# theoad/ot-vae-lightning

Measured on AMD Instinct MI355X. Metric: training images/sec (whole node) + OT-loss rel-err vs CPU ref, higher is better.
Workload: dtype f32; 1 GPU; MNIST-32 CNN VAE (capacity 8, latent 128x1x1, residual=add) + GaussianPrior(loss_coeff=0.1): fwd+bwd+Adam + latent Gaussian statistics update, hipGraph replay; per_gpu_batch=1024, global_batch=1024, parallelism=single GPU

## Files before the change

ot_vae_lightning_amd/csrc/attention.hip:

```cpp
#include "common.h"
#include <type_traits>

#define LOG2E 1.4426950408889634f
#define LN2 0.6931471805599453f
#define EXP2(x) __builtin_amdgcn_exp2f(x)
#define ATTN_LDS_FLOATS 16384
#ifndef OTVAE_ATTN_PACK
#define OTVAE_ATTN_PACK 1
#endif
#define ATTN_BOUND_GAP 64.0f

template <int C>
__device__ __forceinline__ float dotc(const float (&a)[C], const float* __restrict__ b) {
    float s = 0.f;
#pragma unroll
    for (int c = 0; c < C; ++c) s = fmaf(a[c], b[c], s);
    return s;
}

template <int C>
struct Rec {
    static constexpr int KV = 2 * C;
    static constexpr int QG = (2 * C + 2 + 3) & ~3;
};

__device__ __forceinline__ int adiv(int k, int d, float inv_d) {
    return k < (1 << 22) ? (int)(((float)k + 0.5f) * inv_d) : k / d;
}

template <int C, int STRIDE = 2 * C>
__device__ __forceinline__ void stage_kv(float* __restrict__ sm, const float* __restrict__ qkv, long slice0, int nsl, int T,
                                         int H) {
    const int HC = H * C, W3 = 3 * HC;
    const int per = T * 2 * C;
    const float inv_per = 1.0f / (float)per, inv_h = 1.0f / (float)H;
    const int n0 = (int)(slice0 / H), h0 = (int)(slice0 - (long)n0 * H);
    const int total = nsl * per, NT = blockDim.x;
    for (int e0 = threadIdx.x; e0 < total; e0 += 4 * NT) {
        float val[4];
        int dst[4];
#pragma unroll
        for (int u = 0; u < 4; ++u) {
            const int e = e0 + u * NT;
            dst[u] = -1;
            val[u] = 0.f;
            if (e < total) {
                const int sl = adiv(e, per, inv_per), r = e - sl * per;
                const int t = r / (2 * C), j = r - t * 2 * C;
                const int which = j / C, c = j - which * C;
                const int hs = h0 + sl;
                const int dn = adiv(hs, H, inv_h);
                const long n = n0 + dn;
                const int h = hs - dn * H;
                dst[u] = STRIDE == 2 * C ? e : (sl * T + t) * STRIDE + j;
// ... 134 lines not shown
                    const float wv = w[ci * ncols + j];
#pragma unroll
                    for (int t = 0; t < 4; ++t) a[t][j] = fmaf(xr[t], wv, a[t][j]);
                }
            }
        }
        store(tg * 4, col, a);
    }
}

template <int C, int KVS, int NC, bool QREC, bool AFF = false>
__device__ __forceinline__ void stage_qkv(float* __restrict__ kvrec, float* __restrict__ qd, int qstride, float qmul,
                                          const float* __restrict__ xs, const float* __restrict__ wl, int ntok, int T, int H,
                                          float* __restrict__ gq, const float* __restrict__ sc = nullptr,
                                          const float* __restrict__ sh = nullptr) {
    const int HC = H * C, W3 = 3 * HC;
    token_gemm<NC, AFF>(xs, ntok, HC, wl, W3, [&](int t0_, int col0, const float (&a)[4][NC]) {
        const int img = t0_ / T, tt = t0_ - img * T;
#pragma unroll
        for (int j = 0; j < NC; ++j) {
            const int col = col0 + j;
            const int part = col / HC, hc = col - part * HC;
            const int h_ = hc / C, c_ = hc - h_ * C;
            float* dst;
            int stride;
            float mul = 1.f;
            if (part == 0) {
                if constexpr (QREC) {
                    dst = qd + ((size_t)(img * H + h_) * T + tt) * qstride + c_;
                    stride = qstride;
                } else {
                    dst = qd + (size_t)t0_ * HC + hc;
                    stride = HC;
                }
                mul = qmul;
            } else {
                dst = kvrec + ((size_t)(img * H + h_) * T + tt) * KVS + (part - 1) * C + c_;
                stride = KVS;
            }
#pragma unroll
            for (int t = 0; t < 4; ++t) dst[t * stride] = a[t][j] * mul;
        }
        if (gq) {
#pragma unroll
            for (int t = 0; t < 4; ++t) {
                float* g = gq + (size_t)(t0_ + t) * W3 + col0;
                if constexpr (NC == 2) *reinterpret_cast<float2*>(g) = make_float2(a[t][0], a[t][1]);
                else g[0] = a[t][0];
            }
        }
    }, sc, sh);
}

template <int NC>
__device__ __forceinline__ void column_sums_to_partial(double (&s1)[NC], double (&s2)[NC], double* __restrict__ red, int HC,
                                                       double* __restrict__ partial) {
    const int cg = HC / NC;
    for (int m = cg; m < 64; m <<= 1) {
#pragma unroll
        for (int j = 0; j < NC; ++j) {
            s1[j] += __shfl_xor(s1[j], m, 64);
            s2[j] += __shfl_xor(s2[j], m, 64);
        }
    }
    const int lane = threadIdx.x & 63, wave = threadIdx.x >> 6, nw = blockDim.x >> 6;
    if (lane < cg) {
#pragma unroll
        for (int j = 0; j < NC; ++j) {
            red[(wave * 2 + 0) * HC + lane * NC + j] = s1[j];
            red[(wave * 2 + 1) * HC + lane * NC + j] = s2[j];
        }
    }
    __syncthreads();
    if ((int)threadIdx.x < 2 * HC) {
        const int which = threadIdx.x / HC, cc = threadIdx.x - which * HC;
        double t = red[which * HC + cc];
        for (int w = 1; w < nw; ++w) t += red[(w * 2 + which) * HC + cc];
        bn_stat_out(partial, which, HC, cc, gridDim.x, blockIdx.x, t);
    }
}

template <int NC>
__device__ __forceinline__ void stage_project(const float* __restrict__ xs, const float* __restrict__ wl, double* __restrict__ red,
                                              int ntok, int HC, float* __restrict__ yg, const float* __restrict__ rg,
                                              double* __restrict__ stat_partial) {
    double s1[NC], s2[NC];
#pragma unroll
    for (int j = 0; j < NC; ++j) s1[j] = s2[j] = 0.;
    token_gemm<NC>(xs, ntok, HC, wl, HC, [&](int t0_, int col0, const float (&a)[4][NC]) {
#pragma unroll
        for (int t = 0; t < 4; ++t) {
            const size_t o = (size_t)(t0_ + t) * HC + col0;
            float v[NC];
#pragma unroll
            for (int j = 0; j < NC; ++j) v[j] = a[t][j];
            if (rg) {
                if constexpr (NC == 2) {
                    const float2 rv = *reinterpret_cast<const float2*>(rg + o);
                    v[0] += rv.x, v[1] += rv.y;
                } else v[0] += rg[o];
            }
            if constexpr (NC == 2) *reinterpret_cast<float2*>(yg + o) = make_float2(v[0], v[1]);
            else yg[o] = v[0];
#pragma unroll
            for (int j = 0; j < NC; ++j) {
                s1[j] += (double)v[j];
                s2[j] += (double)v[j] * (double)v[j];
            }
        }
    });
    if (stat_partial) column_sums_to_partial<NC>(s1, s2, red, HC, stat_partial);
}

template <int C, int QPT, bool AUX, bool FUSED>
__device__ __forceinline__ void attn_fwd_body(float* __restrict__ sm, const float* __restrict__ qkv, int N, int T, int H, int SPB,
                                              float* __restrict__ out, float* __restrict__ lse, float* __restrict__ aux,
                                              float qk_scale, const AttnStage& sg) {
    constexpr int KVS = FwdRec<C, AUX>::KV;
    const int HC = H * C, W3 = 3 * HC;
    const int TPS = T / QPT;
    const long total = (long)N * H;
    const long slice0 = (long)blockIdx.x * SPB;
    const int nsl = (int)min((long)SPB, total - slice0);
    float* qs = sm + (size_t)SPB * T * KVS;
    float* xs = qs + (size_t)SPB * T * C;
    float* wl = xs + (size_t)SPB * T * C;
    float* wpl = wl + 3 * HC * HC;
    const int ntok = FUSED ? nsl / H * T : 0;
    const size_t tok0 = FUSED ? (size_t)(slice0 / H) * T : 0;
    if constexpr (FUSED) {
        if (sg.fold.slots) {
            __shared__ __align__(16) float bn_tab[2][32];
            bn_fold_prologue(sg.fold, HC, bn_tab[0], bn_tab[1], blockIdx.x == 0);
            stage_input_tile(xs, sg.x + tok0 * HC, ntok * HC, HC, bn_tab[0], bn_tab[1]);
        } else {
            stage_input_tile(xs, sg.x + tok0 * HC, ntok * HC, HC, sg.scale, sg.shift);
        }
        stage_weights(wl, sg.wqkv, HC * W3);
        stage_weights(wpl, sg.wproj, HC * HC);
        __syncthreads();
        float* gq = sg.qkv ? sg.qkv + tok0 * W3 : nullptr;
        if (HC & 1) stage_qkv<C, KVS, 1, false>(sm, qs, 0, 1.f, xs, wl, ntok, T, H, gq);
        else stage_qkv<C, KVS, 2, false>(sm, qs, 0, 1.f, xs, wl, ntok, T, H, gq);
    } else {
        stage_kv<C, KVS>(sm, qkv, slice0, nsl, T, H);
    }
    __syncthreads();
    const int sl = adiv((int)threadIdx.x, TPS, 1.0f / (float)TPS);
    const bool active = sl < nsl;
    const int t0 = (threadIdx.x - sl * TPS) * QPT;
    long n;
    int h;
    {
        const int bn0 = (int)(slice0 / H), bh0 = (int)(slice0 - (long)bn0 * H);
        const int hs = bh0 + sl;
        const int dn = adiv(hs, H, 1.0f / (float)H);
        n = bn0 + dn;
        h = hs - dn * H;
    }
    const float inv_c = LOG2E * qk_scale;
    float* kv = sm + (size_t)(active ? sl : 0) * T * KVS;

    constexpr int NA = AUX ? C * C + C : 1;
    float q[QPT][C], acc[QPT][C], mx[QPT], l[QPT], am[QPT][NA];
    __shared__ float red[4];
    const bool fast = slice_reduce_ok(TPS);
    float vbar[C], kmax = -INFINITY, kmin = INFINITY, knorm = 0.f;
#pragma unroll
    for (int c = 0; c < C; ++c) vbar[c] = 0.f;
    if (fast) {
#pragma unroll
        for (int i = 0; i < QPT; ++i) {
            const float* r = kv + (size_t)(t0 + i) * KVS;
            if constexpr (AUX) {
#pragma unroll
                for (int c = 0; c < C; ++c) vbar[c] += r[C + c];
            }
            if constexpr (C == 1) {
                kmax = fmaxf(kmax, r[0]);
                kmin = fminf(kmin, r[0]);
            } else {
                float s2 = 0.f;
#pragma unroll
                for (int c = 0; c < C; ++c) s2 = fmaf(r[c], r[c], s2);
                knorm = fmaxf(knorm, s2);
            }
        }
        if constexpr (C > 1) knorm = __builtin_sqrtf(slice_reduce<1>(knorm, TPS, red));
        if constexpr (AUX) {
#pragma unroll
            for (int c = 0; c < C; ++c) vbar[c] = slice_reduce<0>(vbar[c], TPS, red);
        }
// ... 121 lines not shown
                f2 sc = nm2[j];
#pragma unroll
                for (int c = 0; c < C; ++c) sc = __builtin_elementwise_fma(q2[j][c], (f2){kk[c], kk[c]}, sc);
                scs[2 * j] = sc.x;
                scs[2 * j + 1] = sc.y;
            }
        } else {
#pragma unroll
            for (int i = 0; i < QPT; ++i) {
                float sc = -mx[i];
#pragma unroll
                for (int c = 0; c < C; ++c) sc = fmaf(q[i][c], kk[c], sc);
                scs[i] = sc;
            }
        }
#pragma unroll
        for (int i = 0; i < QPT; ++i) {
            const float p = EXP2(scs[i]);
            l[i] += p;
#pragma unroll
            for (int c = 0; c < C; ++c) acc[i][c] = fmaf(p, vv[c], acc[i][c]);
            if constexpr (AUX) {
#pragma unroll
                for (int c = 0; c < C; ++c) am[i][C * C + c] = fmaf(p, kk[c], am[i][C * C + c]);
#pragma unroll
                for (int a = 0; a < C * C; ++a) am[i][a] = fmaf(p, uu[a], am[i][a]);
            }
        }
    }
#pragma unroll
    for (int i = 0; i < QPT; ++i) {
        const float rl = 1.f / l[i];
        float* o = out + (n * T + t0 + i) * HC + h * C;
#pragma unroll
        for (int c = 0; c < C; ++c) {
            o[c] = acc[i][c] * rl;
            if constexpr (FUSED) xs[((size_t)img_l * T + t0 + i) * HC + h * C + c] = acc[i][c] * rl;
        }
        lse[(n * H + h) * T + t0 + i] = mx[i] * LN2 + __logf(l[i]);
        if constexpr (AUX) {
            float* ao = aux + (((size_t)n * H + h) * T + t0 + i) * (C * C);
#pragma unroll
            for (int c2 = 0; c2 < C; ++c2)
#pragma unroll
                for (int c = 0; c < C; ++c)
                    ao[c2 * C + c] = (am[i][c2 * C + c] - (acc[i][c2] * rl - vbar[c2]) * am[i][C * C + c]) * rl;
        }
    }
    }
    if constexpr (FUSED) {
        __syncthreads();
        float* yg = sg.y + tok0 * HC;
        const float* rg = sg.residual ? sg.residual + tok0 * HC : nullptr;
        double* red = reinterpret_cast<double*>(qs);
        if (HC & 1) stage_project<1>(xs, wpl, red, ntok, HC, yg, rg, sg.stat_partial);
        else stage_project<2>(xs, wpl, red, ntok, HC, yg, rg, sg.stat_partial);
    }
}

template <int C, int QPT, bool AUX>
__global__ __launch_bounds__(256) void attn_fwd_kernel(const float* __restrict__ qkv, int N, int T, int H, int SPB,
                                                       float* __restrict__ out, float* __restrict__ lse,
                                                       float* __restrict__ aux, float qk_scale) {
    extern __shared__ __align__(16) float sm[];
    attn_fwd_body<C, QPT, AUX, false>(sm, qkv, N, T, H, SPB, out, lse, aux, qk_scale, AttnStage{});
}

template <int C, int QPT, bool AUX>
__global__ __launch_bounds__(256) void attn_stage_fwd_kernel(AttnStage sg, int N, int T, int H, int SPB, float* __restrict__ out,
                                                             float* __restrict__ lse, float* __restrict__ aux, float qk_scale) {
    extern __shared__ __align__(16) float sm[];
    attn_fwd_body<C, QPT, AUX, true>(sm, nullptr, N, T, H, SPB, out, lse, aux, qk_scale, sg);
}

struct AttnStageBwd {
    const float* gy;
    const float* wproj;
    const float* wqkv;
    const float* x;
    const float* mean;
    const float* invstd;
    float* gv;
    double* bn_partial;
    const float* scale;
    const float* shift;
    int direct;
};

__device__ __forceinline__ void stage_weights_t(float* __restrict__ dst, const float* __restrict__ src, int rows, int cols) {
    const int n = rows * cols;
    const float inv_cols = 1.0f / (float)cols;
    for (int i0 = threadIdx.x; i0 < n; i0 += 8 * blockDim.x) {
        float v[8];
#pragma unroll
        for (int u = 0; u < 8; ++u) {
            const int i = i0 + u * blockDim.x;
            v[u] = i < n ? src[i] : 0.f;
        }
#pragma unroll
        for (int u = 0; u < 8; ++u) {
            const int i = i0 + u * blockDim.x;
            if (i < n) {
                const int r = adiv(i, cols, inv_cols), c = i - r * cols;
                dst[c * rows + r] = v[u];
            }
        }
    }
}

template <int C, int QPT, bool AUX, bool FUSED>
__device__ __forceinline__ void attn_bwd_body(float* __restrict__ sm, const float* __restrict__ qkv, const float* __restrict__ out,
                                              const float* __restrict__ lse_g, const float* __restrict__ gout,
                                              const float* __restrict__ aux, int N, int T, int H, int SPB,
                                              float* __restrict__ gqkv, float qk_scale, const AttnStageBwd& sg) {
    constexpr int RKV = Rec<C>::KV, RQG = Rec<C>::QG;
    const int HC = H * C, W3 = 3 * HC;
    const int TPS = T / QPT;
    const long total = (long)N * H;
    const long slice0 = (long)blockIdx.x * SPB;
    const int nsl = (int)min((long)SPB, total - slice0);
    float* s_kv = sm;
    float* s_qg = sm + (size_t)SPB * T * RKV;
    float* wl = s_qg + (size_t)SPB * T * RQG;
    float* wql = wl + HC * HC;
    float* wq3 = wql + 3 * HC * HC;
    float* s_red = wl + ((7 * HC * HC + 3) & ~3);
    float* s_gy = s_red + 16 * HC;
    float* s_x = s_gy + (size_t)SPB * T * C;
    const bool recompute = FUSED && qkv == nullptr;
    const bool direct = FUSED && sg.direct != 0;
    const int ntok = FUSED ? nsl / H * T : 0;
    const size_t tok0 = FUSED ? (size_t)(slice0 / H) * T : 0;
    const float inv_c = qk_scale;
    if (!recompute) stage_kv<C>(s_kv, qkv, slice0, nsl, T, H);
    if constexpr (FUSED) {
        if (recompute) {
            if (!direct) stage_input_tile(s_x, sg.x + tok0 * HC, ntok * HC, HC, sg.scale, sg.shift);
            stage_weights(wq3, sg.wqkv, HC * W3);
        }
        if (!direct) stage_weights(s_gy, sg.gy + tok0 * HC, ntok * HC);
        stage_weights_t(wl, sg.wproj, HC, HC);
        stage_weights_t(wql, sg.wqkv, HC, W3);
        __syncthreads();
        auto put = [&](int t0_, int col0, const auto& a) {
            constexpr int NC_ = sizeof(a[0]) / sizeof(float);
            const int img = t0_ / T, tt = t0_ - img * T;
#pragma unroll
            for (int j = 0; j < NC_; ++j) {
                const int hc = col0 + j, h_ = hc / C, c_ = hc - h_ * C;
                float* dst = s_qg + ((size_t)(img * H + h_) * T + tt) * RQG + C + c_;
#pragma unroll
                for (int t = 0; t < 4; ++t) dst[t * RQG] = a[t][j];
            }
        };
        const float* gy_rows = direct ? sg.gy + tok0 * HC : s_gy;
        if (HC & 1) token_gemm<1>(gy_rows, ntok, HC, wl, HC, put);
        else token_gemm<2>(gy_rows, ntok, HC, wl, HC, put);
        if (recompute) {
            const float* x_rows = direct ? sg.x + tok0 * HC : s_x;
            if (direct && sg.scale) {
                if (HC & 1) stage_qkv<C, RKV, 1, true, true>(s_kv, s_qg, RQG, inv_c, x_rows, wq3, ntok, T, H, nullptr, sg.scale, sg.shift);
                else stage_qkv<C, RKV, 2, true, true>(s_kv, s_qg, RQG, inv_c, x_rows, wq3, ntok, T, H, nullptr, sg.scale, sg.shift);
            } else {
                if (HC & 1) stage_qkv<C, RKV, 1, true>(s_kv, s_qg, RQG, inv_c, x_rows, wq3, ntok, T, H, nullptr);
                else stage_qkv<C, RKV, 2, true>(s_kv, s_qg, RQG, inv_c, x_rows, wq3, ntok, T, H, nullptr);
            }
        }
        __syncthreads();
    }
    const float inv_t = 1.0f / (float)T, inv_hq = 1.0f / (float)H;
    const int qn0 = (int)(slice0 / H), qh0 = (int)(slice0 - (long)qn0 * H);
#pragma unroll 2
    for (int it = threadIdx.x; it < nsl * T; it += blockDim.x) {
        const int sl = adiv(it, T, inv_t), t = it - sl * T;
        const int hs = qh0 + sl;
        const int dn = adiv(hs, H, inv_hq);
        const long n = qn0 + dn;
        const int h = hs - dn * H;
        float* r = s_qg + (size_t)it * RQG;
        const float* qp = qkv + (n * T + t) * W3 + h * C;
        const float* gp = FUSED ? r + C : gout + (n * T + t) * HC + h * C;
        const float* op = out + (n * T + t) * HC + h * C;
        float d = 0.f;
#pragma unroll
        for (int c = 0; c < C; ++c) {
            const float g = gp[c];
            if (!recompute) r[c] = qp[c] * inv_c;
            if constexpr (!FUSED) r[C + c] = g;
            d = fmaf(g, op[c], d);
        }
        r[2 * C] = lse_g[(n * H + h) * T + t] * LOG2E;
        r[2 * C + 1] = d;
    }
    __syncthreads();
    const int sl = adiv((int)threadIdx.x, TPS, 1.0f / (float)TPS);
    const bool active = sl < nsl;
    if constexpr (!FUSED) {
        if (!active) return;
    }
    const int t0 = (threadIdx.x - sl * TPS) * QPT;
    float res[FUSED ? QPT : 1][3][C];
    long n;
    int h;
    {
        const int bn0 = (int)(slice0 / H), bh0 = (int)(slice0 - (long)bn0 * H);
        const int hs = bh0 + sl;
        const int dn = adiv(hs, H, 1.0f / (float)H);
        n = bn0 + dn;
        h = hs - dn * H;
    }
    const float* kv = s_kv + (size_t)sl * T * RKV;
    const float* qg = s_qg + (size_t)sl * T * RQG;
    float dqv[QPT][C];
    constexpr bool PHB = !AUX;
    float dl_new[PHB ? QPT : 1];
// ... 271 lines not shown
                __builtin_amdgcn_fence(__ATOMIC_ACQUIRE, "wavefront");
                float4* o = reinterpret_cast<float4*>(gqkv + (n * T + (t0 - (int)(threadIdx.x & 63) * 4)) * 3);
                const float4* r4 = reinterpret_cast<const float4*>(w);
#pragma unroll
                for (int k4 = 0; k4 < 3; ++k4) o[k4 * 64 + (threadIdx.x & 63)] = r4[k4 * 64 + (threadIdx.x & 63)];
                return;
            }
        }
        if constexpr (FUSED) {
#pragma unroll
            for (int i = 0; i < QPT; ++i)
#pragma unroll
                for (int c = 0; c < C; ++c) res[i][0][c] = dqv[i][c], res[i][1][c] = dk[i][c], res[i][2][c] = dv[i][c];
        } else {
#pragma unroll
        for (int i = 0; i < QPT; ++i) {
            float* o = gqkv + (n * T + t0 + i) * W3 + h * C;
#pragma unroll
            for (int c = 0; c < C; ++c) {
                o[c] = dqv[i][c];
                o[HC + c] = dk[i][c];
                o[2 * HC + c] = dv[i][c];
            }
        }
        }
    }
    }
    if constexpr (FUSED) {
        __syncthreads();
        float* dq_s = sm;
        if (active) {
            const int img_l = (int)(n - slice0 / H);
#pragma unroll
            for (int i = 0; i < QPT; ++i) {
                float* o = dq_s + ((size_t)img_l * T + t0 + i) * W3 + h * C;
#pragma unroll
                for (int c = 0; c < C; ++c) o[c] = res[i][0][c], o[HC + c] = res[i][1][c], o[2 * HC + c] = res[i][2][c];
            }
        }
        __syncthreads();
        {
            float* g = gqkv + tok0 * W3;
            const int nq = ntok * W3;
            if ((nq & 3) == 0 && (reinterpret_cast<uintptr_t>(g) & 15) == 0) {
                for (int i = threadIdx.x * 4; i < nq; i += blockDim.x * 4) *reinterpret_cast<float4*>(g + i) = *reinterpret_cast<const float4*>(dq_s + i);
            } else {
                for (int i = threadIdx.x; i < nq; i += blockDim.x) g[i] = dq_s[i];
            }
        }
        float* gvg = sg.gv + tok0 * HC;
        const float* xg = sg.x ? sg.x + tok0 * HC : nullptr;
        auto project = [&](auto nc_tag) {
            constexpr int NC_ = decltype(nc_tag)::value;
            double s1[NC_], s2[NC_];
#pragma unroll
            for (int j = 0; j < NC_; ++j) s1[j] = s2[j] = 0.;
            float mu[NC_], is[NC_];
            const int col_t = (threadIdx.x % (HC / NC_)) * NC_;
#pragma unroll
            for (int j = 0; j < NC_; ++j) mu[j] = sg.mean ? sg.mean[col_t + j] : 0.f, is[j] = sg.mean ? sg.invstd[col_t + j] : 0.f;
            token_gemm<NC_>(dq_s, ntok, W3, wql, HC, [&](int t0_, int col0, const float (&a)[4][NC_]) {
#pragma unroll
                for (int t = 0; t < 4; ++t) {
                    const size_t o = (size_t)(t0_ + t) * HC + col0;
                    if constexpr (NC_ == 2) *reinterpret_cast<float2*>(gvg + o) = make_float2(a[t][0], a[t][1]);
                    else gvg[o] = a[t][0];
                    if (sg.mean) {
#pragma unroll
                        for (int j = 0; j < NC_; ++j) {
                            const float xv = xg[o + j];
                            s1[j] += (double)a[t][j];
                            s2[j] += (double)a[t][j] * (double)((xv - mu[j]) * is[j]);
                        }
                    }
                }
            });
            if (sg.bn_partial) column_sums_to_partial<NC_>(s1, s2, reinterpret_cast<double*>(s_red), HC, sg.bn_partial);
        };
        if (HC & 1) project(std::integral_constant<int, 1>{});
        else project(std::integral_constant<int, 2>{});
    }
}

template <int C, int QPT, bool AUX>
__global__ __launch_bounds__(256) void attn_bwd_kernel(const float* __restrict__ qkv, const float* __restrict__ out,
                                                       const float* __restrict__ lse_g, const float* __restrict__ gout,
                                                       const float* __restrict__ aux, int N, int T, int H, int SPB,
                                                       float* __restrict__ gqkv, float qk_scale) {
    extern __shared__ __align__(16) float sm[];
    attn_bwd_body<C, QPT, AUX, false>(sm, qkv, out, lse_g, gout, aux, N, T, H, SPB, gqkv, qk_scale, AttnStageBwd{});
}

template <int C, int QPT, bool AUX>
__global__ __launch_bounds__(256) void attn_stage_bwd_kernel(AttnStageBwd sg, const float* __restrict__ qkv, const float* __restrict__ out,
                                                             const float* __restrict__ lse_g, const float* __restrict__ aux, int N, int T,
                                                             int H, int SPB, float* __restrict__ gqkv, float qk_scale) {
    extern __shared__ __align__(16) float sm[];
    attn_bwd_body<C, QPT, AUX, true>(sm, qkv, out, lse_g, nullptr, aux, N, T, H, SPB, gqkv, qk_scale, sg);
}


__global__ __launch_bounds__(256) void attn_t1_fwd_kernel(const float* __restrict__ qkv, int N, int H, int C, float scale,
                                                          float* __restrict__ out, float* __restrict__ lse) {
    const int HC = H * C;
    const int i = blockIdx.x * 256 + threadIdx.x;
    if (i < N * HC) {
        const int n = i / HC, hc = i - n * HC;
        out[i] = qkv[(size_t)n * 3 * HC + 2 * HC + hc];
    }
    if (i < N * H) {
        const int n = i / H, h = i - n * H;
        const float* q = qkv + (size_t)n * 3 * HC + h * C;
        float s = 0.f;
        for (int c = 0; c < C; ++c) s = fmaf(q[c], q[HC + c], s);
        lse[i] = s * scale;
    }
}

__global__ __launch_bounds__(256) void attn_t1_bwd_kernel(const float* __restrict__ gout, int N, int HC, float* __restrict__ gqkv) {
    const int i = blockIdx.x * 256 + threadIdx.x;
    if (i >= N * 3 * HC) return;
    const int n = i / (3 * HC), j = i - n * 3 * HC;
    gqkv[i] = j >= 2 * HC ? gout[(size_t)n * HC + j - 2 * HC] : 0.f;
}

static int pick_qpt(int T, int C) { return (T >= 256 && T % 4 == 0 && C <= 4) ? 4 : 1; }
static int pick_spb(int T, int qpt, int floats_per_key) {
    static const int cap_env = getenv("OTVAE_ATTN_SPB") ? atoi(getenv("OTVAE_ATTN_SPB")) : 0;
    int tps = T / qpt;
    int spb = 256 / tps;
    int cap = ATTN_LDS_FLOATS / (T * floats_per_key);
    if (spb > cap) spb = cap;
    if (cap_env > 0 && spb > cap_env && (cap_env * tps) % 64 == 0) spb = cap_env;
    return spb;
}
static int attn_threads(int spb, int T, int qpt) { return imax(64, (spb * (T / qpt) + 63) / 64 * 64); }

#define ATTN_C_SWITCH(C_, MACRO)                                                                              \
    switch (C_) {                                                                                             \
        case 1: MACRO(1); break;                                                                              \
        case 2: MACRO(2); break;                                                                              \
        case 3: MACRO(3); break;                                                                              \
        case 4: MACRO(4); break;                                                                              \
        case 6: MACRO(6); break;                                                                              \
        case 8: MACRO(8); break;                                                                              \
        case 12: MACRO(12); break;                                                                            \
        case 16: MACRO(16); break;                                                                            \
        case 32: MACRO(32); break;                                                                            \
        default:                                                                                              \
            otvae_set_error("attention: head width C=%d not instantiated (1,2,3,4,6,8,12,16,32)", C_);        \
            return OTVAE_EUNSUPPORTED;                                                                        \
// ... 24 lines not shown
extern "C" int otvae_attn_fwd_scaled(const float* qkv, int N, int T, int H, int C, float scale, float* out, float* lse, float* aux,
                                     void* stream) {
    OTVAE_REQUIRE(qkv && out && lse, "otvae_attn_fwd: NULL tensor");
    OTVAE_REQUIRE(scale > 0.f, "otvae_attn_fwd: scale must be positive");
    if (T == 1 && N > 0 && H > 0 && C > 0) {
        attn_t1_fwd_kernel<<<cdiv((int64_t)N * H * C, 256), 256, 0, (hipStream_t)stream>>>(qkv, N, H, C, scale, out, lse);
        OTVAE_CHECK_LAUNCH("otvae_attn_fwd(T=1)");
        return OTVAE_OK;
    }
    int qpt, spb;
    if (C > 2) aux = nullptr;
    const int rkv = aux ? ((2 * C + C * C + 3) & ~3) : 2 * C;
    int rc = attn_check("otvae_attn_fwd", N, T, H, C, rkv, &qpt, &spb);
    if (rc) return rc;
    hipStream_t st = (hipStream_t)stream;
    const int grid = cdiv((int64_t)N * H, spb), nthr = attn_threads(spb, T, qpt);
    const size_t lds = (size_t)spb * T * rkv * sizeof(float);
#define FWD_K(CC)                                                                                   \
    do {                                                                                            \
        if (qpt == 4) {                                                                             \
            if constexpr (CC <= 2) {                                                                \
                if (aux) attn_fwd_kernel<CC, 4, true><<<grid, nthr, lds, st>>>(qkv, N, T, H, spb, out, lse, aux, scale); \
                else attn_fwd_kernel<CC, 4, false><<<grid, nthr, lds, st>>>(qkv, N, T, H, spb, out, lse, nullptr, scale); \
            } else if constexpr (CC <= 4) attn_fwd_kernel<CC, 4, false><<<grid, nthr, lds, st>>>(qkv, N, T, H, spb, out, lse, nullptr, scale); \
            else { otvae_set_error("otvae_attn_fwd: T >= 256 with head width %d > 4 unsupported", CC); return OTVAE_EUNSUPPORTED; } \
        } else {                                                                                    \
            if constexpr (CC <= 2) {                                                                \
                if (aux) attn_fwd_kernel<CC, 1, true><<<grid, nthr, lds, st>>>(qkv, N, T, H, spb, out, lse, aux, scale); \
                else attn_fwd_kernel<CC, 1, false><<<grid, nthr, lds, st>>>(qkv, N, T, H, spb, out, lse, nullptr, scale); \
            } else attn_fwd_kernel<CC, 1, false><<<grid, nthr, lds, st>>>(qkv, N, T, H, spb, out, lse, nullptr, scale); \
        }                                                                                           \
    } while (0)
    ATTN_C_SWITCH(C, FWD_K)
#undef FWD_K
    OTVAE_CHECK_LAUNCH("otvae_attn_fwd");
    return OTVAE_OK;
}

#define ATTN_STAGE_LDS_FLOATS 24576
template <auto Kernel>
static int stage_lds_ok(size_t lds) {
    static size_t granted = 64 * 1024;
    if (lds <= granted) return OTVAE_OK;
    const hipError_t e = hipFuncSetAttribute(reinterpret_cast<const void*>(Kernel), hipFuncAttributeMaxDynamicSharedMemorySize,
                                             ATTN_STAGE_LDS_FLOATS * sizeof(float));
    if (e != hipSuccess) {
        otvae_set_error("otvae_attn_stage_fwd: %zu bytes of LDS refused: %s", lds, hipGetErrorString(e));
        return OTVAE_ELAUNCH;
    }
    granted = ATTN_STAGE_LDS_FLOATS * sizeof(float);
    return OTVAE_OK;
}
static inline bool attn_aligned16(const void* p) { return ((uintptr_t)p & 15) == 0; }
static int attn_stage_shape(int N, int T, int H, int C, bool aux, bool backward, int* qpt, int* spb, int* grid, int* nthr, size_t* lds,
                            bool quiet, int* direct = nullptr) {
    const int HC = H * C;
#define STAGE_NO(...)                                  \
    do {                                               \
        if (!quiet) otvae_set_error(__VA_ARGS__);      \
        return OTVAE_EUNSUPPORTED;                     \
    } while (0)
    if (N <= 0 || T <= 1 || H <= 0 || C <= 0) STAGE_NO("otvae_attn_stage: bad sizes / T == 1");
    if (T % 4 != 0 || HC > 32 || (HC & (HC - 1)) != 0) STAGE_NO("otvae_attn_stage: needs T %% 4 == 0 and a power-of-two width <= 32 (T=%d, width=%d)", T, HC);
    switch (C) {
        case 1: case 2: case 3: case 4: case 6: case 8: case 12: case 16: case 32: break;
        default: STAGE_NO("otvae_attn_stage: head width %d not instantiated", C);
    }
    *qpt = pick_qpt(T, C);
    const int tps = T / *qpt;
    if (tps > 256 || (*qpt == 4 && C > 4)) STAGE_NO("otvae_attn_stage: T = %d with head width %d unsupported", T, C);
    const int rkv = aux ? ((2 * C + C * C + 3) & ~3) : 2 * C;
    const int rec_slice = T * (2 * C + ((2 * C + 2 + 3) & ~3));
    const int bw_floats = ((7 * HC * HC + 3) & ~3) + 16 * HC;
    static const int direct_env = getenv("OTVAE_ATTN_STAGE_DIRECT") ? atoi(getenv("OTVAE_ATTN_STAGE_DIRECT")) : 1;
    if (direct) *direct = 0;
    if (backward && direct && direct_env) {
        const int s3 = imin(256 / tps, (ATTN_STAGE_LDS_FLOATS - bw_floats) / rec_slice) / H * H;
        const size_t third = 160 * 1024 / 3;
        if (s3 >= H && ((size_t)s3 * (rec_slice + 2 * T * C) + bw_floats) * sizeof(float) > third &&
            ((size_t)s3 * rec_slice + bw_floats) * sizeof(float) <= third)
            *direct = 1;
    }
    const int per_slice = backward ? rec_slice + ((direct && *direct) ? 0 : 2 * T * C) : T * (rkv + 2 * C);
    const int wfloats = backward ? bw_floats : 4 * HC * HC;
    int s = imin(256 / tps, (ATTN_STAGE_LDS_FLOATS - wfloats) / per_slice) / H * H;
    if (s < H) STAGE_NO("otvae_attn_stage: the %d heads of an image do not fit one workgroup (T=%d)", H, T);
    while ((int64_t)N * H / s < 256 && s % (2 * H) == 0 && ((s / 2) * tps) % 64 == 0 && (s / 2 / H) * T >= 16) s /= 2;
    if ((s / H) * T < 16) STAGE_NO("otvae_attn_stage: fewer than 16 tokens per workgroup");
    *spb = s;
    *grid = (int)cdiv((int64_t)N * H, s);
    *nthr = attn_threads(s, T, *qpt);
    *lds = ((size_t)s * per_slice + wfloats) * sizeof(float);
#undef STAGE_NO
    return OTVAE_OK;
}

extern "C" int otvae_attn_stage_plan(int N, int T, int H, int C, int need_aux, int* stat_rows) {
    int qpt, spb, grid, nthr;
    size_t lds;
    int rc = attn_stage_shape(N, T, H, C, need_aux && C <= 2, false, &qpt, &spb, &grid, &nthr, &lds, true);
    if (rc) return rc;
    if (stat_rows) *stat_rows = grid;
    return OTVAE_OK;
}

extern "C" int otvae_attn_stage_bwd_plan(int N, int T, int H, int C, int* bn_rows) {
    int qpt, spb, grid, nthr;
    size_t lds;
    int direct;
    int rc = attn_stage_shape(N, T, H, C, false, true, &qpt, &spb, &grid, &nthr, &lds, true, &direct);
    if (rc) return rc;
    if (bn_rows) *bn_rows = grid;
    return OTVAE_OK;
}

static int attn_stage_fwd_impl(const float* x, const float* scale, const float* shift, const float* wqkv, const float* wproj,
                               const float* residual, int N, int T, int H, int C, float qk_scale, float* qkv, float* out, float* lse,
                               float* aux, float* y, double* stat_partial, const BnFold& fold, void* stream);

extern "C" int otvae_attn_stage_fwd(const float* x, const float* scale, const float* shift, const float* wqkv, const float* wproj,
                                    const float* residual, int N, int T, int H, int C, float qk_scale, float* qkv, float* out, float* lse,
                                    float* aux, float* y, double* stat_partial, void* stream) {
    return attn_stage_fwd_impl(x, scale, shift, wqkv, wproj, residual, N, T, H, C, qk_scale, qkv, out, lse, aux, y, stat_partial, BnFold{},
                               stream);
}

extern "C" int otvae_attn_stage_fwd_fold(const float* x, const otvae_bn_fold* fold, const float* scale, const float* shift,
                                         const float* wqkv, const float* wproj, const float* residual, int N, int T, int H, int C,
                                         float qk_scale, float* qkv, float* out, float* lse, float* aux, float* y, double* stat_partial,
                                         void* stat_slots, int stat_nslots, void* stream) {
    OTVAE_REQUIRE(!(stat_partial && stat_slots), "otvae_attn_stage_fwd_fold: statistics go to partials OR to slots");
    OTVAE_REQUIRE_SLOTS("otvae_attn_stage_fwd_fold", stat_slots, stat_nslots);
    BnFold f = {};
    if (fold)
        if (int rc = bn_fold_from_abi("otvae_attn_stage_fwd_fold", *fold, H * C, &f)) return rc;
    return attn_stage_fwd_impl(x, scale, shift, wqkv, wproj, residual, N, T, H, C, qk_scale, qkv, out, lse, aux, y,
                               stat_slots ? bn_tag_slots(stat_slots, stat_nslots) : stat_partial, f, stream);
}

static int attn_stage_fwd_impl(const float* x, const float* scale, const float* shift, const float* wqkv, const float* wproj,
                               const float* residual, int N, int T, int H, int C, float qk_scale, float* qkv, float* out, float* lse,
                               float* aux, float* y, double* stat_partial, const BnFold& fold, void* stream) {
    OTVAE_REQUIRE(x && wqkv && wproj && out && lse && y, "otvae_attn_stage_fwd: NULL tensor");
    OTVAE_REQUIRE((scale == nullptr) == (shift == nullptr), "otvae_attn_stage_fwd: scale/shift must come together");
    OTVAE_REQUIRE(qk_scale > 0.f, "otvae_attn_stage_fwd: scale must be positive");
    if (C > 2) aux = nullptr;
// ... 144 lines not shown
```

Before: 395,700 images/s.

## Make fused attention stage kernels persistent, staging weights once per workgroup

The fused attention stage forward and backward kernels now loop over slice groups with a grid-stride loop. Weights, the transposed weights and the BN scale/shift are staged into LDS once per workgroup instead of once per group, and the column statistics accumulate across groups before a single reduction. The grid is capped at the resident workgroup count from an occupancy query when the weight footprint rivals the per-group token tile. It also vectorizes the weight transpose and restricts the direct backward path to T >= 256. The cost is less parallelism, extra barriers per group and a host-side occupancy cache.

```diff
diff --git a/ot_vae_lightning_amd/csrc/attention.hip b/ot_vae_lightning_amd/csrc/attention.hip
--- a/ot_vae_lightning_amd/csrc/attention.hip
+++ b/ot_vae_lightning_amd/csrc/attention.hip
@@ -1,5 +1,7 @@
 #include "common.h"
+#include <mutex>
 #include <type_traits>
+#include <vector>
 
 #define LOG2E 1.4426950408889634f
 #define LN2 0.6931471805599453f
@@ -240,8 +242,11 @@
     }, sc, sh);
 }
 
+struct StageSums {
+    double s1[2], s2[2];
+};
 template <int NC>
-__device__ __forceinline__ void column_sums_to_partial(double (&s1)[NC], double (&s2)[NC], double* __restrict__ red, int HC,
+__device__ __forceinline__ void column_sums_to_partial(double (&s1)[2], double (&s2)[2], double* __restrict__ red, int HC,
                                                        double* __restrict__ partial) {
     const int cg = HC / NC;
     for (int m = cg; m < 64; m <<= 1) {
@@ -269,12 +274,10 @@
 }
 
 template <int NC>
-__device__ __forceinline__ void stage_project(const float* __restrict__ xs, const float* __restrict__ wl, double* __restrict__ red,
-                                              int ntok, int HC, float* __restrict__ yg, const float* __restrict__ rg,
-                                              double* __restrict__ stat_partial) {
-    double s1[NC], s2[NC];
-#pragma unroll
-    for (int j = 0; j < NC; ++j) s1[j] = s2[j] = 0.;
+__device__ __forceinline__ void stage_project(const float* __restrict__ xs, const float* __restrict__ wl, int ntok, int HC,
+                                              float* __restrict__ yg, const float* __restrict__ rg, StageSums& sums) {
+    double (&s1)[2] = sums.s1;
+    double (&s2)[2] = sums.s2;
     token_gemm<NC>(xs, ntok, HC, wl, HC, [&](int t0_, int col0, const float (&a)[4][NC]) {
 #pragma unroll
         for (int t = 0; t < 4; ++t) {
@@ -297,18 +300,18 @@
             }
         }
     });
-    if (stat_partial) column_sums_to_partial<NC>(s1, s2, red, HC, stat_partial);
 }
 
 template <int C, int QPT, bool AUX, bool FUSED>
 __device__ __forceinline__ void attn_fwd_body(float* __restrict__ sm, const float* __restrict__ qkv, int N, int T, int H, int SPB,
                                               float* __restrict__ out, float* __restrict__ lse, float* __restrict__ aux,
-                                              float qk_scale, const AttnStage& sg) {
+                                              float qk_scale, const AttnStage& sg, long group, const float* __restrict__ bn_sc,
+                                              const float* __restrict__ bn_sh, StageSums& sums) {
     constexpr int KVS = FwdRec<C, AUX>::KV;
     const int HC = H * C, W3 = 3 * HC;
     const int TPS = T / QPT;
     const long total = (long)N * H;
-    const long slice0 = (long)blockIdx.x * SPB;
+    const long slice0 = group * SPB;
     const int nsl = (int)min((long)SPB, total - slice0);
     float* qs = sm + (size_t)SPB * T * KVS;
     float* xs = qs + (size_t)SPB * T * C;
@@ -317,15 +320,7 @@
     const int ntok = FUSED ? nsl / H * T : 0;
     const size_t tok0 = FUSED ? (size_t)(slice0 / H) * T : 0;
     if constexpr (FUSED) {
-        if (sg.fold.slots) {
-            __shared__ __align__(16) float bn_tab[2][32];
-            bn_fold_prologue(sg.fold, HC, bn_tab[0], bn_tab[1], blockIdx.x == 0);
-            stage_input_tile(xs, sg.x + tok0 * HC, ntok * HC, HC, bn_tab[0], bn_tab[1]);
-        } else {
-            stage_input_tile(xs, sg.x + tok0 * HC, ntok * HC, HC, sg.scale, sg.shift);
-        }
-        stage_weights(wl, sg.wqkv, HC * W3);
-        stage_weights(wpl, sg.wproj, HC * HC);
+        stage_input_tile(xs, sg.x + tok0 * HC, ntok * HC, HC, bn_sc, bn_sh);
         __syncthreads();
         float* gq = sg.qkv ? sg.qkv + tok0 * W3 : nullptr;
         if (HC & 1) stage_qkv<C, KVS, 1, false>(sm, qs, 0, 1.f, xs, wl, ntok, T, H, gq);
@@ -553,9 +548,9 @@
         __syncthreads();
         float* yg = sg.y + tok0 * HC;
         const float* rg = sg.residual ? sg.residual + tok0 * HC : nullptr;
-        double* red = reinterpret_cast<double*>(qs);
-        if (HC & 1) stage_project<1>(xs, wpl, red, ntok, HC, yg, rg, sg.stat_partial);
-        else stage_project<2>(xs, wpl, red, ntok, HC, yg, rg, sg.stat_partial);
+        if (HC & 1) stage_project<1>(xs, wpl, ntok, HC, yg, rg, sums);
+        else stage_project<2>(xs, wpl, ntok, HC, yg, rg, sums);
+        __syncthreads();
     }
 }
 
@@ -564,14 +559,37 @@
                                                        float* __restrict__ out, float* __restrict__ lse,
                                                        float* __restrict__ aux, float qk_scale) {
     extern __shared__ __align__(16) float sm[];
-    attn_fwd_body<C, QPT, AUX, false>(sm, qkv, N, T, H, SPB, out, lse, aux, qk_scale, AttnStage{});
+    StageSums sums;
+    attn_fwd_body<C, QPT, AUX, false>(sm, qkv, N, T, H, SPB, out, lse, aux, qk_scale, AttnStage{}, blockIdx.x, nullptr, nullptr, sums);
 }
 
 template <int C, int QPT, bool AUX>
 __global__ __launch_bounds__(256) void attn_stage_fwd_kernel(AttnStage sg, int N, int T, int H, int SPB, float* __restrict__ out,
                                                              float* __restrict__ lse, float* __restrict__ aux, float qk_scale) {
     extern __shared__ __align__(16) float sm[];
-    attn_fwd_body<C, QPT, AUX, true>(sm, nullptr, N, T, H, SPB, out, lse, aux, qk_scale, sg);
+    constexpr int KVS = FwdRec<C, AUX>::KV;
+    const int HC = H * C;
+    __shared__ __align__(16) float bn_tab[2][32];
+    const bool affine = sg.fold.slots || sg.scale;
+    if (sg.fold.slots) {
+        bn_fold_prologue(sg.fold, HC, bn_tab[0], bn_tab[1], blockIdx.x == 0);
+    } else if (sg.scale) {
+        for (int c = threadIdx.x; c < HC; c += blockDim.x) bn_tab[0][c] = sg.scale[c], bn_tab[1][c] = sg.shift[c];
+    }
+    float* wl = sm + (size_t)SPB * T * (KVS + 2 * C);
+    stage_weights(wl, sg.wqkv, 3 * HC * HC);
+    stage_weights(wl + 3 * HC * HC, sg.wproj, HC * HC);
+    __syncthreads();
+    StageSums sums = {{0., 0.}, {0., 0.}};
+    const long groups = ((long)N * H + SPB - 1) / SPB;
+    for (long g = blockIdx.x; g < groups; g += gridDim.x)
+        attn_fwd_body<C, QPT, AUX, true>(sm, nullptr, N, T, H, SPB, out, lse, aux, qk_scale, sg, g, affine ? bn_tab[0] : nullptr,
+                                         bn_tab[1], sums);
+    if (sg.stat_partial) {
+        double* red = reinterpret_cast<double*>(sm + (size_t)SPB * T * KVS);
+        if (HC & 1) column_sums_to_partial<1>(sums.s1, sums.s2, red, HC, sg.stat_partial);
+        else column_sums_to_partial<2>(sums.s1, sums.s2, red, HC, sg.stat_partial);
+    }
 }
 
 struct AttnStageBwd {
@@ -589,44 +607,63 @@
 };
 
 __device__ __forceinline__ void stage_weights_t(float* __restrict__ dst, const float* __restrict__ src, int rows, int cols) {
-    const int n = rows * cols;
-    const float inv_cols = 1.0f / (float)cols;
-    for (int i0 = threadIdx.x; i0 < n; i0 += 8 * blockDim.x) {
-        float v[8];
-#pragma unroll
-        for (int u = 0; u < 8; ++u) {
-            const int i = i0 + u * blockDim.x;
-            v[u] = i < n ? src[i] : 0.f;
-        }
-#pragma unroll
-        for (int u = 0; u < 8; ++u) {
-            const int i = i0 + u * blockDim.x;
-            if (i < n) {
-                const int r = adiv(i, cols, inv_cols), c = i - r * cols;
-                dst[c * rows + r] = v[u];
-            }
-        }
-    }
-}
+    const float inv_rows = 1.0f / (float)rows;
+    if ((cols & 3) == 0 && (reinterpret_cast<uintptr_t>(src) & 15) == 0) {
+        const int n4 = rows * (cols >> 2);
+        for (int e0 = threadIdx.x; e0 < n4; e0 += 4 * blockDim.x) {
+            float4 v[4];
+            int at[4];
+#pragma unroll
+            for (int u = 0; u < 4; ++u) {
+                const int e = e0 + u * blockDim.x;
+                at[u] = -1;
+                if (e < n4) {
+                    const int c4 = adiv(e, rows, inv_rows), r = e - c4 * rows;
+                    v[u] = *reinterpret_cast<const float4*>(src + (size_t)r * cols + c4 * 4);
+                    at[u] = c4 * 4 * rows + r;
+                }
+            }
+#pragma unroll
+            for (int u = 0; u < 4; ++u)
+                if (at[u] >= 0) {
+                    float* d = dst + at[u];
+                    d[0] = v[u].x, d[rows] = v[u].y, d[2 * rows] = v[u].z, d[3 * rows] = v[u].w;
+                }
+        }
+    } else {
+        const int n = rows * cols;
+        for (int i = threadIdx.x; i < n; i += blockDim.x) {
+            const int c = adiv(i, rows, inv_rows), r = i - c * rows;
+            dst[i] = src[(size_t)r * cols + c];
+        }
+    }
+}
+
+struct StageBwdState {
+    const float* sc;
+    const float* sh;
+    float mu[2], is[2];
+    StageSums sums;
+};
 
 template <int C, int QPT, bool AUX, bool FUSED>
 __device__ __forceinline__ void attn_bwd_body(float* __restrict__ sm, const float* __restrict__ qkv, const float* __restrict__ out,
                                               const float* __restrict__ lse_g, const float* __restrict__ gout,
                                               const float* __restrict__ aux, int N, int T, int H, int SPB,
-                                              float* __restrict__ gqkv, float qk_scale, const AttnStageBwd& sg) {
+                                              float* __restrict__ gqkv, float qk_scale, const AttnStageBwd& sg, long group,
+                                              StageBwdState& st) {
     constexpr int RKV = Rec<C>::KV, RQG = Rec<C>::QG;
     const int HC = H * C, W3 = 3 * HC;
     const int TPS = T / QPT;
     const long total = (long)N * H;
-    const long slice0 = (long)blockIdx.x * SPB;
+    const long slice0 = group * SPB;
     const int nsl = (int)min((long)SPB, total - slice0);
     float* s_kv = sm;
     float* s_qg = sm + (size_t)SPB * T * RKV;
     float* wl = s_qg + (size_t)SPB * T * RQG;
     float* wql = wl + HC * HC;
     float* wq3 = wql + 3 * HC * HC;
-    float* s_red = wl + ((7 * HC * HC + 3) & ~3);
-    float* s_gy = s_red + 16 * HC;
+    float* s_gy = wl + ((7 * HC * HC + 3) & ~3) + 16 * HC;
     float* s_x = s_gy + (size_t)SPB * T * C;
     const bool recompute = FUSED && qkv == nullptr;
     const bool direct = FUSED && sg.direct != 0;
@@ -635,13 +672,8 @@
     const float inv_c = qk_scale;
     if (!recompute) stage_kv<C>(s_kv, qkv, slice0, nsl, T, H);
     if constexpr (FUSED) {
-        if (recompute) {
-            if (!direct) stage_input_tile(s_x, sg.x + tok0 * HC, ntok * HC, HC, sg.scale, sg.shift);
-            stage_weights(wq3, sg.wqkv, HC * W3);
-        }
+        if (recompute && !direct) stage_input_tile(s_x, sg.x + tok0 * HC, ntok * HC, HC, st.sc, st.sh);
         if (!direct) stage_weights(s_gy, sg.gy + tok0 * HC, ntok * HC);
-        stage_weights_t(wl, sg.wproj, HC, HC);
-        stage_weights_t(wql, sg.wqkv, HC, W3);
         __syncthreads();
         auto put = [&](int t0_, int col0, const auto& a) {
             constexpr int NC_ = sizeof(a[0]) / sizeof(float);
@@ -659,9 +691,9 @@
         else token_gemm<2>(gy_rows, ntok, HC, wl, HC, put);
         if (recompute) {
             const float* x_rows = direct ? sg.x + tok0 * HC : s_x;
-            if (direct && sg.scale) {
-                if (HC & 1) stage_qkv<C, RKV, 1, true, true>(s_kv, s_qg, RQG, inv_c, x_rows, wq3, ntok, T, H, nullptr, sg.scale, sg.shift);
-                else stage_qkv<C, RKV, 2, true, true>(s_kv, s_qg, RQG, inv_c, x_rows, wq3, ntok, T, H, nullptr, sg.scale, sg.shift);
+            if (direct && st.sc) {
+                if (HC & 1) stage_qkv<C, RKV, 1, true, true>(s_kv, s_qg, RQG, inv_c, x_rows, wq3, ntok, T, H, nullptr, st.sc, st.sh);
+                else stage_qkv<C, RKV, 2, true, true>(s_kv, s_qg, RQG, inv_c, x_rows, wq3, ntok, T, H, nullptr, st.sc, st.sh);
             } else {
                 if (HC & 1) stage_qkv<C, RKV, 1, true>(s_kv, s_qg, RQG, inv_c, x_rows, wq3, ntok, T, H, nullptr);
                 else stage_qkv<C, RKV, 2, true>(s_kv, s_qg, RQG, inv_c, x_rows, wq3, ntok, T, H, nullptr);
@@ -1039,13 +1071,10 @@
         const float* xg = sg.x ? sg.x + tok0 * HC : nullptr;
         auto project = [&](auto nc_tag) {
             constexpr int NC_ = decltype(nc_tag)::value;
-            double s1[NC_], s2[NC_];
-#pragma unroll
-            for (int j = 0; j < NC_; ++j) s1[j] = s2[j] = 0.;
-            float mu[NC_], is[NC_];
-            const int col_t = (threadIdx.x % (HC / NC_)) * NC_;
-#pragma unroll
-            for (int j = 0; j < NC_; ++j) mu[j] = sg.mean ? sg.mean[col_t + j] : 0.f, is[j] = sg.mean ? sg.invstd[col_t + j] : 0.f;
+            double (&s1)[2] = st.sums.s1;
+            double (&s2)[2] = st.sums.s2;
+            const float (&mu)[2] = st.mu;
+            const float (&is)[2] = st.is;
             token_gemm<NC_>(dq_s, ntok, W3, wql, HC, [&](int t0_, int col0, const float (&a)[4][NC_]) {
 #pragma unroll
                 for (int t = 0; t < 4; ++t) {
@@ -1062,10 +1091,10 @@
                     }
                 }
             });
-            if (sg.bn_partial) column_sums_to_partial<NC_>(s1, s2, reinterpret_cast<double*>(s_red), HC, sg.bn_partial);
         };
         if (HC & 1) project(std::integral_constant<int, 1>{});
         else project(std::integral_constant<int, 2>{});
+        __syncthreads();
     }
 }
 
@@ -1075,7 +1104,8 @@
                                                        const float* __restrict__ aux, int N, int T, int H, int SPB,
                                                        float* __restrict__ gqkv, float qk_scale) {
     extern __shared__ __align__(16) float sm[];
-    attn_bwd_body<C, QPT, AUX, false>(sm, qkv, out, lse_g, gout, aux, N, T, H, SPB, gqkv, qk_scale, AttnStageBwd{});
+    StageBwdState st;
+    attn_bwd_body<C, QPT, AUX, false>(sm, qkv, out, lse_g, gout, aux, N, T, H, SPB, gqkv, qk_scale, AttnStageBwd{}, blockIdx.x, st);
 }
 
 template <int C, int QPT, bool AUX>
@@ -1083,7 +1113,35 @@
                                                              const float* __restrict__ lse_g, const float* __restrict__ aux, int N, int T,
                                                              int H, int SPB, float* __restrict__ gqkv, float qk_scale) {
     extern __shared__ __align__(16) float sm[];
-    attn_bwd_body<C, QPT, AUX, true>(sm, qkv, out, lse_g, nullptr, aux, N, T, H, SPB, gqkv, qk_scale, sg);
+    const int HC = H * C;
+    __shared__ __align__(16) float bn_tab[2][32];
+    float* wl = sm + (size_t)SPB * T * (Rec<C>::KV + Rec<C>::QG);
+    float* wql = wl + HC * HC;
+    StageBwdState st = {nullptr, nullptr, {0.f, 0.f}, {0.f, 0.f}, {{0., 0.}, {0., 0.}}};
+    if (qkv == nullptr) {
+        stage_weights(wql + 3 * HC * HC, sg.wqkv, 3 * HC * HC);
+        if (sg.scale) {
+            for (int c = threadIdx.x; c < HC; c += blockDim.x) bn_tab[0][c] = sg.scale[c], bn_tab[1][c] = sg.shift[c];
+            st.sc = bn_tab[0], st.sh = bn_tab[1];
+        }
+    }
+    stage_weights_t(wl, sg.wproj, HC, HC);
+    stage_weights_t(wql, sg.wqkv, HC, 3 * HC);
+    if (sg.mean) {
+        const int nc = (HC & 1) ? 1 : 2, col_t = (threadIdx.x % (HC / nc)) * nc;
+#pragma unroll
+        for (int j = 0; j < 2; ++j)
+            if (j < nc) st.mu[j] = sg.mean[col_t + j], st.is[j] = sg.invstd[col_t + j];
+    }
+    __syncthreads();
+    const long groups = ((long)N * H + SPB - 1) / SPB;
+    for (long g = blockIdx.x; g < groups; g += gridDim.x)
+        attn_bwd_body<C, QPT, AUX, true>(sm, qkv, out, lse_g, nullptr, aux, N, T, H, SPB, gqkv, qk_scale, sg, g, st);
+    if (sg.bn_partial) {
+        double* red = reinterpret_cast<double*>(wl + ((7 * HC * HC + 3) & ~3));
+        if (HC & 1) column_sums_to_partial<1>(st.sums.s1, st.sums.s2, red, HC, sg.bn_partial);
+        else column_sums_to_partial<2>(st.sums.s1, st.sums.s2, red, HC, sg.bn_partial);
+    }
 }
 
 
@@ -1214,6 +1272,74 @@
     return OTVAE_OK;
 }
 static inline bool attn_aligned16(const void* p) { return ((uintptr_t)p & 15) == 0; }
+
+static const void* stage_kernel_ptr(bool backward, int C, int qpt, bool aux) {
+    const void* k = nullptr;
+#define STAGE_PICK(CC)                                                                                                             \
+    do {                                                                                                                           \
+        if (qpt == 4) {                                                                                                            \
+            if constexpr (CC <= 2) {                                                                                               \
+                if (aux) k = backward ? (const void*)&attn_stage_bwd_kernel<CC, 4, true> : (const void*)&attn_stage_fwd_kernel<CC, 4, true>;   \
+                else k = backward ? (const void*)&attn_stage_bwd_kernel<CC, 4, false> : (const void*)&attn_stage_fwd_kernel<CC, 4, false>;     \
+            } else if constexpr (CC <= 4)                                                                                          \
+                k = backward ? (const void*)&attn_stage_bwd_kernel<CC, 4, false> : (const void*)&attn_stage_fwd_kernel<CC, 4, false>;          \
+        } else {                                                                                                                   \
+            if constexpr (CC <= 2) {                                                                                               \
+                if (aux) k = backward ? (const void*)&attn_stage_bwd_kernel<CC, 1, true> : (const void*)&attn_stage_fwd_kernel<CC, 1, true>;   \
+                else k = backward ? (const void*)&attn_stage_bwd_kernel<CC, 1, false> : (const void*)&attn_stage_fwd_kernel<CC, 1, false>;     \
+            } else                                                                                                                 \
+                k = backward ? (const void*)&attn_stage_bwd_kernel<CC, 1, false> : (const void*)&attn_stage_fwd_kernel<CC, 1, false>;          \
+        }                                                                                                                          \
+    } while (0)
+    switch (C) {
+        case 1: STAGE_PICK(1); break;
+        case 2: STAGE_PICK(2); break;
+        case 3: STAGE_PICK(3); break;
+        case 4: STAGE_PICK(4); break;
+        case 6: STAGE_PICK(6); break;
+        case 8: STAGE_PICK(8); break;
+        case 12: STAGE_PICK(12); break;
+        case 16: STAGE_PICK(16); break;
+        case 32: STAGE_PICK(32); break;
+        default: break;
+    }
+#undef STAGE_PICK
+    return k;
+}
+
+static int stage_resident_wgs(const void* kernel, int nthr, size_t lds, int* wgs) {
+    struct Seen { const void* kernel; int nthr; size_t lds; int wgs; };
+    static std::vector<Seen> seen;
+    static std::mutex mu;
+    std::lock_guard<std::mutex> lock(mu);
+    for (const Seen& e : seen)
+        if (e.kernel == kernel && e.nthr == nthr && e.lds == lds) {
+            *wgs = e.wgs;
+            return OTVAE_OK;
+        }
+    if (lds > 64 * 1024) {
+        const hipError_t e = hipFuncSetAttribute(kernel, hipFuncAttributeMaxDynamicSharedMemorySize, ATTN_STAGE_LDS_FLOATS * sizeof(float));
+        if (e != hipSuccess) {
+            otvae_set_error("otvae_attn_stage: %zu bytes of LDS refused: %s", lds, hipGetErrorString(e));
+            return OTVAE_ELAUNCH;
+        }
+    }
+    int dev = 0, cus = 0, per_cu = 0;
+    hipError_t e = hipGetDevice(&dev);
+    if (e == hipSuccess) e = hipDeviceGetAttribute(&cus, hipDeviceAttributeMultiprocessorCount, dev);
+    if (e == hipSuccess) e = hipOccupancyMaxActiveBlocksPerMultiprocessor(&per_cu, kernel, nthr, lds);
+    if (e != hipSuccess || cus <= 0 || per_cu <= 0) {
+        otvae_set_error("otvae_attn_stage: occupancy query failed (%s; %d units x %d workgroups)", hipGetErrorString(e), cus, per_cu);
+        return OTVAE_ELAUNCH;
+    }
+    seen.push_back({kernel, nthr, lds, cus * per_cu});
+    *wgs = cus * per_cu;
+    return OTVAE_OK;
+}
+
+#ifndef OTVAE_ATTN_STAGE_WALK
+#define OTVAE_ATTN_STAGE_WALK 1
+#endif
 static int attn_stage_shape(int N, int T, int H, int C, bool aux, bool backward, int* qpt, int* spb, int* grid, int* nthr, size_t* lds,
                             bool quiet, int* direct = nullptr) {
     const int HC = H * C;
@@ -1236,7 +1362,7 @@
     const int bw_floats = ((7 * HC * HC + 3) & ~3) + 16 * HC;
     static const int direct_env = getenv("OTVAE_ATTN_STAGE_DIRECT") ? atoi(getenv("OTVAE_ATTN_STAGE_DIRECT")) : 1;
     if (direct) *direct = 0;
-    if (backward && direct && direct_env) {
+    if (backward && direct && direct_env && T >= 256) {
         const int s3 = imin(256 / tps, (ATTN_STAGE_LDS_FLOATS - bw_floats) / rec_slice) / H * H;
         const size_t third = 160 * 1024 / 3;
         if (s3 >= H && ((size_t)s3 * (rec_slice + 2 * T * C) + bw_floats) * sizeof(float) > third &&
@@ -1254,6 +1380,18 @@
     *nthr = attn_threads(s, T, *qpt);
     *lds = ((size_t)s * per_slice + wfloats) * sizeof(float);
 #undef STAGE_NO
+    const bool walk = OTVAE_ATTN_STAGE_WALK == 2 || (OTVAE_ATTN_STAGE_WALK == 1 && wfloats >= (s / H) * T * HC);
+    if (walk) {
+        const void* kernels[2] = {stage_kernel_ptr(backward, C, *qpt, !backward && aux),
+                                  backward && C <= 2 ? stage_kernel_ptr(true, C, *qpt, true) : nullptr};
+        for (const void* k : kernels) {
+            if (!k) continue;
+            int wgs = 0;
+            const int rc = stage_resident_wgs(k, *nthr, *lds, &wgs);
+            if (rc) return rc;
+            if (*grid > wgs) *grid = wgs;
+        }
+    }
     return OTVAE_OK;
 }
 
```

Result: slower. 388,200 images/s (-1.9%).
